# JuliaLinearAlgebra/AlgebraicMultigrid.jl

Hardware: AMD Instinct MI355X
Metric: V-cycle unknowns/sec + fine-level SpMV GB/s (% HBM peak), 3-D Poisson 256^3 (higher is better)
Workload: dtype f64

## Files before the change

### algebraicmultigrid.jl_amd/_libs.py

```python
import ctypes as C
import os

_HERE = os.path.dirname(os.path.abspath(__file__))
SETUP_SO = os.path.join(_HERE, "libamgsetup.so")
HIP_SO = os.path.join(_HERE, "libamghip.so")
HIP_F32_SO = os.path.join(_HERE, "libamghip_f32.so")

i32p = C.POINTER(C.c_int32)
f64p = C.POINTER(C.c_double)
i64 = C.c_int64
vp = C.c_void_p


class AMGError(RuntimeError):
    pass


class amgs_options(C.Structure):
    _fields_ = [("theta", C.c_double), ("max_levels", C.c_int32), ("max_coarse", C.c_int32),
                ("hermitian", C.c_int32), ("sa_omega", C.c_double), ("sa_improve_iters", C.c_int32),
                ("sa_B_is_vector", C.c_int32)]


class amgh_smoother_t(C.Structure):
# ... 141 lines not shown
    L.amgh_dev_upload.argtypes = [C.c_int, vp, vp, i64]
    L.amgh_dev_download.argtypes = [C.c_int, vp, vp, i64]
    L.amgh_dev_sync.argtypes = [C.c_int]
    L.amgh_stream.restype = vp
    L.amgh_stream.argtypes = [vp]
    L.amgh_timer_begin.argtypes = [vp]
    L.amgh_timer_end.argtypes = [vp, C.POINTER(C.c_double)]
    L.amgh_bench_op.argtypes = [vp, C.c_int, C.c_int, C.c_int, C.c_int, C.POINTER(C.c_double)]
    L.amgh_debug_chain_timing.argtypes = [C.c_int, vp]
    L.amgh_debug_merged_sweep_host.argtypes = [i64, i64, vp, vp, vp, C.c_int, C.c_int, C.c_double, vp, vp]
    L.amgh_debug_bw_poll_giveups.argtypes = [vp, C.c_int]
    L.amgh_debug_bw_mode.argtypes = [vp, C.c_int]
    L.amgh_debug_bw_dict.argtypes = [vp, C.c_int]
    L.amgh_debug_bw_late.argtypes = [vp, C.c_int]
    L.amgh_debug_coded_ops.argtypes = [vp, C.c_int]
    L.amgh_debug_set_sell_stream.argtypes = [C.c_int, i64, C.c_int]
    L.amgh_debug_sell_stream_launches.argtypes = [vp, C.c_int, C.c_int]
    L.amgh_debug_sell_stream_padded.argtypes = [vp, C.c_int, C.c_int]
    L.amgh_debug_sell_stream_padded.restype = i64
    L.amgh_debug_csr_sell.argtypes = [vp, C.c_int]
    L.amgh_debug_csr_sell.restype = i64
    L.amgh_debug_csr_sell_launches.argtypes = [vp]
    L.amgh_debug_csr_sell_apply.argtypes = [vp, C.c_int, vp, vp, vp]
    L.amgh_debug_bw_sweep_host.argtypes = [i64, vp, vp, vp, C.c_int, C.c_int, C.c_double, vp, vp, vp]
    L.amgh_debug_bw_dict_sweep_host.argtypes = [i64, vp, vp, vp, C.c_int, C.c_int, vp, vp, vp]
    L.amgh_debug_set_tunable.argtypes = [C.c_char_p, C.c_int]
    L.amgh_debug_get_tunable.argtypes = [C.c_char_p, C.POINTER(C.c_int)]
    L.amgh_profile_enable.argtypes = [vp, C.c_int]
    L.amgh_profile_read.argtypes = [vp, vp, C.c_int]
    L.amgh_set_use_graph.argtypes = [vp, C.c_int]


def _bind_dist(L):
    i64p = C.POINTER(i64)
    L.amgh_dist_rccl_available.argtypes = []
    L.amgh_dist_unique_id.argtypes = [vp]
    L.amgh_dist_create_rccl.argtypes = [C.POINTER(vp), C.c_int, C.c_int, C.c_int, vp]
    L.amgh_local_group_create.argtypes = [C.POINTER(vp), C.c_int]
    L.amgh_local_group_destroy.argtypes = [vp]
    L.amgh_local_group_destroy.restype = None
    L.amgh_local_group_abort.argtypes = [vp]
    L.amgh_local_group_abort.restype = None
    L.amgh_dist_create_local.argtypes = [C.POINTER(vp), C.c_int, C.c_int, vp]
    L.amgh_dist_create_ipc.argtypes = [C.POINTER(vp), C.c_int, C.c_int, C.c_int, C.c_char_p]
    L.amgh_dist_destroy.argtypes = [vp]
    L.amgh_dist_destroy.restype = None
# ... 93 lines not shown
```

### algebraicmultigrid.jl_amd/csrc/hip/amghip.hip

```cpp
#include "amghip_internal.hpp"
#include "gs_schedule.hpp"
#include "csr_ops.hpp"
#include "chebyshev.hpp"
#include "gmres_kernels.hpp"
#include "pcg_block_kernels.hpp"
#include "dist_pcg_kernels.hpp"

namespace {

constexpr int64_t kGraphAutoRows = 65536;

struct Level {
  int64_t n = 0, nc = 0;
  amgh_csr A, S, P, R;
  bool has_S = false;
  amgh_smoother_t pre{}, post{};
  real *res = nullptr, *cx = nullptr, *cb = nullptr, *tmp = nullptr;
  real* cheb_d = nullptr;
  ChebSide cheb[2];
  const ChebSide& cheb_of(const amgh_smoother_t& s) const { return &s == &post ? cheb[1] : cheb[0]; }
  real* il = nullptr;
  amgh_csr* smat() { return has_S ? &S : &A; }
  amgh_csr Pp, Rp;
  bool lo_ok = false;
// ... 1306 lines not shown
      if (!L->lo_ok || !L->Rp.rowptr || L->Rp.nrows < (1 << 18)) continue;
      if (hipMemsetAsync(L->res, 0, sizeof(real) * L->n, h->stream) != hipSuccess) return -1001;
      double ms[2] = {0, 0};
      int rc = AMGH_OK;
      for (int v = 0; v < 2 && rc == AMGH_OK; ++v) {
        L->Rp.xcd_map = v == 1;
        rc = csr_apply(&L->Rp, M_SPMV, L->res, nullptr, L->cb, h->stream, 1);
        if (rc == AMGH_OK && hipEventRecord(h->t0, h->stream) != hipSuccess) rc = -1001;
        for (int r = 0; r < 4 && rc == AMGH_OK; ++r) rc = csr_apply(&L->Rp, M_SPMV, L->res, nullptr, L->cb, h->stream, 1);
        float t = 0.f;
        if (rc == AMGH_OK && (hipEventRecord(h->t1, h->stream) != hipSuccess || hipEventSynchronize(h->t1) != hipSuccess ||
                              hipEventElapsedTime(&t, h->t0, h->t1) != hipSuccess)) rc = -1001;
        ms[v] = t;
      }
      L->Rp.xcd_map = false;
      RC_TRY(rc);
      L->Rp.xcd_map = ms[1] < 0.93 * ms[0];
      if (getenv("AMGH_VERBOSE")) fprintf(stderr, "[amghip] n=%lld restriction: %.3f ms, XCD-contiguous %.3f ms -> %s\n", (long long)L->n, ms[0] / 4, ms[1] / 4, L->Rp.xcd_map ? "XCD-contiguous" : "plain");
    }
  if (h->nrhs == 1)
    for (Level* L : h->levels) {
      GsSchedule* g = L->smat()->gs;
      const bool cd = g_stream_code != 0;
      if (!(L->lo_ok && g && g->nblk == 0)) {
        for (amgh_csr* M : {&L->A, &L->R, &L->P})
          if (M->rowptr) { RC_TRY(sell_build(M->rowptr, cd ? M->cc.ccol : nullptr, M->col, M->val, M->nrows, M->nnz, &M->sc, h->stream)); ws += M->sc.bytes; }
        continue;
      }
      if (!g->rowptr || g->compacted) continue;
      RC_TRY(sell_build(g->rowptr, cd ? L->lo_cc.ccol : nullptr, g->col, L->lo_val ? L->lo_val : g->val, L->n, g->nnz, &L->lo_sc, h->stream));
      RC_TRY(sell_build(L->Rp.rowptr, cd ? L->Rp.cc.ccol : nullptr, L->Rp.col, L->Rp.val, L->Rp.nrows, L->Rp.nnz, &L->Rp.sc, h->stream));
      RC_TRY(sell_build(L->Pp.rowptr, cd ? L->Pp.cc.ccol : nullptr, L->Pp.col, L->Pp.val, L->Pp.nrows, L->Pp.nnz, &L->Pp.sc, h->stream));
      if (L->n >= (1 << 18) && g_sell_min_rows >= ((int64_t)1 << 18)) {
        real* ty = nullptr;
        RC_TRY(dev_alloc(&ty, L->n));
        int rc = AMGH_OK;
        if (hipMemsetAsync(ty, 0, sizeof(real) * L->n, h->stream) != hipSuccess || hipMemsetAsync(L->res, 0, sizeof(real) * L->n, h->stream) != hipSuccess ||
            hipMemsetAsync(L->cx, 0, sizeof(real) * L->nc, h->stream) != hipSuccess) rc = -1001;
        const real* val = L->lo_val ? L->lo_val : g->val;
        auto run = [&](int which) -> int {
          if (which == AMGH_OP_A) return raw_apply(M_RESID, g->rowptr, g->col, val, L->n, L->res, L->n, L->res, L->n, ty, L->n, h->stream, 1, &L->lo_cc, &L->lo_sc);
          if (which == AMGH_OP_R) return csr_apply(&L->Rp, M_SPMV, L->res, nullptr, L->cb, h->stream, 1, true);
          return raw_apply(M_ADD, L->Pp.rowptr, L->Pp.col, L->Pp.val, L->n, L->cx, L->nc, nullptr, 0, ty, L->n, h->stream, 1, &L->Pp.cc, &L->Pp.sc);
        };
        const int keep = g_sell_stream;
        for (int which : {AMGH_OP_A, AMGH_OP_R, AMGH_OP_P}) {
          SellCols* sc = which == AMGH_OP_A ? &L->lo_sc : which == AMGH_OP_R ? &L->Rp.sc : &L->Pp.sc;
          if (!sc->w || (which == AMGH_OP_R ? L->Rp.nrows : L->n) < (1 << 18)) continue;
          double ms[2] = {0, 0};
          for (int v = 0; v < 2 && rc == AMGH_OK; ++v) {
            g_sell_stream = v;
            rc = run(which);
            if (rc == AMGH_OK && hipEventRecord(h->t0, h->stream) != hipSuccess) rc = -1001;
            for (int r = 0; r < 4 && rc == AMGH_OK; ++r) rc = run(which);
            float t = 0.f;
            if (rc == AMGH_OK && (hipEventRecord(h->t1, h->stream) != hipSuccess || hipEventSynchronize(h->t1) != hipSuccess ||
                                  hipEventElapsedTime(&t, h->t0, h->t1) != hipSuccess)) rc = -1001;
            ms[v] = t;
          }
          sc->launches = 0;
          if (rc != AMGH_OK) break;
          if (getenv("AMGH_VERBOSE")) fprintf(stderr, "[amghip] n=%lld operator %d: csr_stream_kernel %.3f ms, sliced-ELL %.3f ms\n", (long long)L->n, which, ms[0] / 4, ms[1] / 4);
          if (!(ms[1] < 0.97 * ms[0])) sc->free_dev();
        }
        g_sell_stream = keep;
        if (hipStreamSynchronize(h->stream) != hipSuccess && rc == AMGH_OK) rc = -1001;
        hipFree(ty);
        RC_TRY(rc);
      }
      ws += L->lo_sc.bytes + L->Rp.sc.bytes + L->Pp.sc.bytes;
      if (getenv("AMGH_VERBOSE"))
        fprintf(stderr, "[amghip] n=%lld sliced-ELL padded / entries: A %.3f  R %.3f  P %.3f (0: not taken)\n", (long long)L->n, (double)L->lo_sc.padded / std::max<int64_t>(1, g->nnz),
                (double)L->Rp.sc.padded / std::max<int64_t>(1, L->Rp.nnz), (double)L->Pp.sc.padded / std::max<int64_t>(1, L->Pp.nnz));
    }
  if (gs_trim() && g_stream_code && g_trim_coded) {
    HIP_TRY(hipStreamSynchronize(h->stream));
    for (Level* L : h->levels) {
      for (amgh_csr* M : {&L->Rp, &L->Pp})
        if (M->cc.ccol && M->col && M->val) {
          hipFree(M->col); hipFree(M->val); M->col = nullptr; M->val = nullptr;
          M->bytes -= M->nnz * kEntB;
        }
      amgh_csr* S = L->smat();
      GsSchedule* g = S->gs;
      if (L->lo_cc.ccol && g && g->bw.on && g->bw.flow.on && !g->bw.rec && g->segs.empty() && !g->mf && !g->mb && g->col && g->val) {
        hipFree(g->col); hipFree(g->val); g->col = nullptr; g->val = nullptr;
// ... 1059 lines not shown
  return sc ? (sc->w ? sc->padded : 0) : -1;
}

int64_t amgh_debug_csr_sell(amgh_csr_t* op, int coded) {
  if (!op) return AMGH_EINVAL;
  HIP_TRY(hipSetDevice(op->device));
  if (coded && !op->cc.ccol) {
    RC_TRY(code_values(op->col, op->val, op->nrows, op->ncols, op->nnz, &op->cc, nullptr, 1));
    op->bytes += op->cc.bytes;
  }
  RC_TRY(sell_build(op->rowptr, coded ? op->cc.ccol : nullptr, op->col, op->val, op->nrows, op->nnz, &op->sc, nullptr));
  op->bytes += op->sc.bytes;
  return op->sc.w ? op->sc.padded : 0;
}
int amgh_debug_csr_sell_apply(amgh_csr_t* op, int mode, const real* x_d, const real* b_d, real* y_d) {
  if (!op || !x_d || !y_d || mode < M_SPMV || mode > M_ADD || (mode == M_RESID && !b_d)) return AMGH_EINVAL;
  HIP_TRY(hipSetDevice(op->device));
  RC_TRY(csr_apply(op, mode, x_d, b_d, y_d, nullptr, 1, true));
  HIP_TRY(hipDeviceSynchronize());
  return AMGH_OK;
}
int amgh_debug_csr_sell_launches(const amgh_csr_t* op) { return op ? (int)(op->sc.launches & 0x7fffffffu) : -1; }

int amgh_debug_chain_timing(int enable, unsigned long long* out8) {
  if (enable && !g_chain_tim) {
    HIP_TRY(hipMalloc((void**)&g_chain_tim, 8 * sizeof(unsigned long long)));
    HIP_TRY(hipMemset(g_chain_tim, 0, 8 * sizeof(unsigned long long)));
  }
  if (out8 && g_chain_tim) {
    HIP_TRY(hipDeviceSynchronize());
    HIP_TRY(hipMemcpy(out8, g_chain_tim, 8 * sizeof(unsigned long long), hipMemcpyDeviceToHost));
    HIP_TRY(hipMemset(g_chain_tim, 0, 8 * sizeof(unsigned long long)));
  }
  if (!enable && g_chain_tim) { hipFree(g_chain_tim); g_chain_tim = nullptr; }
  return AMGH_OK;
}

int amgh_profile_enable(amgh_t* h, int on) {
  if (!h) return AMGH_EINVAL;
  h->profile = on != 0;
  return AMGH_OK;
}
int amgh_profile_read(amgh_t* h, double* out, int reset) {
  if (!h || !out) return AMGH_EINVAL;
  RC_TRY(prof_flush(h));
  const int L1 = (int)h->levels.size() + 1;
// ... 19 lines not shown
```

### algebraicmultigrid.jl_amd/csrc/hip/amghip_internal.hpp

```cpp
#pragma once
#include "amghip_kernels.hpp"
#include "gs_blocks.hpp"
#include "gs_flow.hpp"

#include <algorithm>
#include <chrono>
#include <cmath>
#include <cstdio>
#include <cstring>
#include <atomic>
#include <mutex>
#include <string>
#include <system_error>
#include <thread>
#include <utility>
#include <vector>

#include "../../../include/amghip.h"

using namespace amgh;

#define HIP_TRY(expr)                                   \
  do {                                                  \
    hipError_t e_ = (expr);                             \
// ... 280 lines not shown
    hipFree(bw.flow.fd); hipFree(bw.flow.srec); hipFree(bw.flow.aux); hipFree(bw.flow.fl_mb); hipFree(bw.flow.fl_slot); hipFree(bw.flow.mbox);
    hipFree(bw.flow.xaux); hipFree(bw.flow.xfl_mb); hipFree(bw.flow.xfl_slot); hipFree(bw.flow.xlist);
    hipFree(bw.flow.crec); hipFree(bw.flow.dict); hipFree(bw.flow.dict_ent);
    bw = Bw();
    hipFree(d_lvl_ptr); hipFree(rowptr); hipFree(col); hipFree(val);
    hipFree(perm); hipFree(dpos); if (!diag_shared) hipFree(diag);
    hipFree(rowmeta); hipFree(desc); hipFree(bp); hipFree(xp); hipFree(permx);
    d_lvl_ptr = rowptr = col = perm = dpos = nullptr; val = diag = bp = xp = nullptr; rowmeta = desc = nullptr; permx = nullptr;
  }
};

}

#include "dev_scan.hpp"

struct CodedCols {
  uint32_t* ccol = nullptr; real* vtab = nullptr; int n = 0;
  int64_t bytes = 0;
  void free_dev() { hipFree(ccol); hipFree(vtab); ccol = nullptr; vtab = nullptr; n = 0; bytes = 0; }
};

constexpr int kSellCapPct = 130, kSellCapPlainPct = 110;
constexpr int kSellLongSteps = 12;
struct SellCols {
  uint32_t* w = nullptr; real* v = nullptr; uint2* slice = nullptr; uint8_t* len8 = nullptr;
  int64_t nslices = 0, padded = 0, bytes = 0;
  unsigned launches = 0;
  void free_dev() { hipFree(w); hipFree(v); hipFree(slice); hipFree(len8); w = nullptr; v = nullptr; slice = nullptr; len8 = nullptr; nslices = padded = bytes = 0; }
};

struct amgh_csr {
  CodedCols cc;
  SellCols sc;
  bool cc_tried = false;
  bool xcd_map = false;
  int device = 0;
  int64_t nrows = 0, ncols = 0, nnz = 0;
  int32_t* rowptr = nullptr;
  int32_t* col = nullptr;
  real* val = nullptr;
  int32_t* dpos = nullptr;
  real* diag = nullptr;
  GsSchedule* gs = nullptr;
  int gs_nrhs_hint = 0;
  uint32_t pipe_epoch = 0; const void* pipe_rmbox = nullptr; int pipe_grid = 0;
  int64_t bytes = 0;
};

namespace {

int g_gs_block_pipe = 1;
// ... 2 lines not shown
int g_gs_bigslot = 1;
int g_gs_merge = 16;
int g_jacobi_zero = 1;
int g_rhs_il = 1;
int g_gs_tiny = 1;
int g_gs_wave_quad = 1;
int g_gs_bw = 1;
int g_gs_bw_rows = 512;
int g_gs_bw_flow = 1;
int g_gs_bw_spin = 0;
int g_gs_bw_skip_pub = -1;
int g_gs_bw_nc = -1;
int g_gs_bw_nrhs = 1;
int g_gs_bw_chain = 1;
int g_stream_code = 1;
int g_trim_coded = 1;
int g_gs_bw_inorder = 0;
int g_gs_bw_dict = 1;
int g_gs_bw_relay = 3;
int g_gs_flow_xzero = 1;
int g_gs_flow_perm_io = 1;
int g_sell_stream = 1;
int64_t g_sell_min_rows = (int64_t)1 << 18;
int g_sell_cap_pct = 0;
unsigned int g_perm_io_sweeps[2] = {0, 0};
int g_gs_bw_two_min_rows = 200000;
int g_gs_sell = 1;
int g_gs_lean = -1;
int g_gs_ept = 0;
int g_gs_lpr = 0;
int g_gs_il = 1;
int g_pcg_fused = 1;
int g_tail_dense_rows = 6144;
int g_tail_dense = 1;
int g_gs_dense_blk = 4096;
int g_gs_dense_tri = 1;
int g_gs_block_inverse = 1;

std::atomic<unsigned long long> g_sched_epoch{0};

unsigned long long* g_chain_tim = nullptr;

constexpr int kChainWidth = 1024;

__global__ void find_diag_kernel(const int32_t* rowptr, const int32_t* col, const real* val, int n,
                                 int32_t* dpos, real* diag) {
// ... 58 lines not shown
```

### algebraicmultigrid.jl_amd/csrc/hip/amghip_kernels.hpp

```cpp
#pragma once
#include <hip/hip_runtime.h>
#include <stdint.h>

#ifndef AMGH_REAL
#define AMGH_REAL double
#endif

namespace amgh {

using real = AMGH_REAL;

constexpr int kWave = 64;
constexpr int kThreads = 256;
constexpr int kNumXcd = 8;

enum StreamMode : int {
  M_SPMV = 0,
  M_RESID = 1,
  M_ADD = 2,
  M_JACOBI = 3,
  M_GS = 4,
  M_SOR = 5,
  M_CHEB1 = 6,
  M_CHEB = 7
// ... 251 lines not shown
          a.y[i] = (gb[q] - acc[q]) / d;
        } else {
          a.y[i] = (1.0 - a.omega) * a.y[i] + (a.omega / d) * (gb[q] - acc[q]);
        }
      }
    }
  }
}

using DefaultCfg = StreamCfg<1024, 1024, 8192, 4, false, false>;

struct SellStreamArgs {
  const uint32_t* w;
  const real* v;
  const uint2* slice;
  const uint8_t* len;
  const int32_t* rowptr;
  const real* vtab;
  int32_t vtab_n;
  int32_t nrows, nslices;
  const real* x;
  const real* b;
  real* y;
};
template <int MODE, bool CODED, int B>
__global__ __launch_bounds__(kThreads) void sell_stream_kernel(SellStreamArgs a) {
  static_assert(MODE == M_SPMV || MODE == M_RESID || MODE == M_ADD, "SpMV-type passes only");
  __shared__ real s_tab[CODED ? kCodeMax : 1];
  if (CODED) {
    if ((int)threadIdx.x < a.vtab_n) s_tab[threadIdx.x] = a.vtab[threadIdx.x];
    __syncthreads();
  }
  const int s = (int)blockIdx.x * (kThreads / kWave) + __builtin_amdgcn_readfirstlane((int)(threadIdx.x >> 6));
  if (s >= a.nslices) return;
  const int lane = threadIdx.x & (kWave - 1);
  const int r = s * kWave + lane;
  const bool live = r < a.nrows;
  int len = 0;
  if (live) len = a.len ? (int)a.len[r] : a.rowptr[r + 1] - a.rowptr[r];
  const uint2 sd = a.slice[s];
  const int nit = (int)sd.y;
  const int64_t base = (int64_t)sd.x * kWave + lane;
  uint32_t w[B];
  real v[B];
#pragma unroll
  for (int e = 0; e < B; ++e) {
    w[e] = 0; v[e] = 0.0;
    if (e < nit) { w[e] = a.w[base + (int64_t)e * kWave]; if (!CODED) v[e] = a.v[base + (int64_t)e * kWave]; }
  }
  real acc = 0.0;
  for (int t = 0; t < nit; t += B) {
    uint32_t wn[B];
    real vn[B];
#pragma unroll
    for (int e = 0; e < B; ++e) {
      wn[e] = 0; vn[e] = 0.0;
      if (t + B + e < nit) { wn[e] = a.w[base + (int64_t)(t + B + e) * kWave]; if (!CODED) vn[e] = a.v[base + (int64_t)(t + B + e) * kWave]; }
    }
    real xv[B];
#pragma unroll
    for (int e = 0; e < B; ++e) {
      const uint32_t c = CODED ? (w[e] & ((1u << kCodeBits) - 1)) : w[e];
      xv[e] = t + e < len ? a.x[c] : (real)0.0;
      if (CODED) v[e] = s_tab[w[e] >> kCodeBits];
    }
#pragma unroll
    for (int e = 0; e < B; ++e)
      if (t + e < len) acc = acc + v[e] * xv[e];
#pragma unroll
    for (int e = 0; e < B; ++e) { w[e] = wn[e]; v[e] = vn[e]; }
  }
  if (!live) return;
  if (MODE == M_SPMV) a.y[r] = acc;
  else if (MODE == M_RESID) a.y[r] = a.b[r] - acc;
  else a.y[r] = a.y[r] + acc;
}
__global__ void sell_steps_kernel(const int32_t* rowptr, int nrows, int nslices, int32_t* steps) {
  const int s = blockIdx.x * blockDim.x + threadIdx.x;
  if (s >= nslices) return;
  const int r1 = min(s * kWave + kWave, nrows);
  int m = 0;
  for (int r = s * kWave; r < r1; ++r) m = max(m, rowptr[r + 1] - rowptr[r]);
  steps[s] = m;
}
__global__ void sell_stream_fill_kernel(const int32_t* rowptr, const uint32_t* w_in, const real* v_in, const uint2* slice, int nrows,
                                        int nslices, uint32_t* w, real* v, uint8_t* len8) {
  const int64_t gid = (int64_t)blockIdx.x * blockDim.x + threadIdx.x;
  const int s = (int)(gid >> 6), lane = (int)(gid & 63);
  if (s >= nslices) return;
  const uint2 sd = slice[s];
  const int r = s * kWave + lane;
  int32_t a0 = 0, len = 0;
  if (r < nrows) { a0 = rowptr[r]; len = rowptr[r + 1] - a0; if (len8) len8[r] = (uint8_t)len; }
  const int64_t base = (int64_t)sd.x * kWave + lane;
  for (int t = 0; t < (int)sd.y; ++t) {
    w[base + (int64_t)t * kWave] = t < len ? w_in[a0 + t] : 0u;
    if (v) v[base + (int64_t)t * kWave] = t < len ? v_in[a0 + t] : (real)0.0;
  }
}

__device__ __forceinline__ real seq_sum_range(const real* s, int lo, int hi, real acc) {
  int j = lo;
  if (hi - j >= 8) {
    real p[8], q[8];
#pragma unroll
    for (int e = 0; e < 8; ++e) p[e] = s[j + e];
    j += 8;
    while (hi - j >= 16) {
#pragma unroll
      for (int e = 0; e < 8; ++e) q[e] = s[j + e];
#pragma unroll
      for (int e = 0; e < 8; ++e) acc += p[e];
#pragma unroll
      for (int e = 0; e < 8; ++e) p[e] = s[j + 8 + e];
#pragma unroll
      for (int e = 0; e < 8; ++e) acc += q[e];
// ... 1656 lines not shown
```

### algebraicmultigrid.jl_amd/csrc/hip/csr_ops.hpp

```cpp
#pragma once
#include <atomic>

namespace {


template <int MODE, class CFG = DefaultCfg, bool CODED = false>
int launch_stream(const StreamArgs& a0, hipStream_t st, int ncolv = 1) {
  const int nrows = a0.row_end - a0.row_begin;
  if (nrows <= 0) return AMGH_OK;
  StreamArgs a = a0;
  a.ncolv = ncolv;
  const int nb = (nrows + CFG::ROWS - 1) / CFG::ROWS;
  const int64_t grid = (CFG::XCD || ncolv > 1) ? (int64_t)((nb + kNumXcd - 1) / kNumXcd) * kNumXcd * ncolv : nb;
  hipLaunchKernelGGL((csr_stream_kernel<MODE, CFG, CODED>), dim3((unsigned)grid), dim3(CFG::THREADS), 0, st, a);
  HIP_TRY(hipGetLastError());
  return AMGH_OK;
}

constexpr int kGsBlockTarget = 256;
constexpr int kGsMinRows = 4;
constexpr int kGsNnzPerWg = 256;
template <int MODE>
int launch_gs_level(const StreamArgs& a, int rows, hipStream_t st, int ncolv = 1) {
  const int width = a.row_end - a.row_begin;
// ... 88 lines not shown
    tab.erase(std::unique(tab.begin(), tab.end()), tab.end());
    if ((int)tab.size() > kCodeMax) ok = false;
    if (pass == 7) ok = false;
  }
  if (rc == AMGH_OK && ok && !tab.empty()) {
    std::vector<real> tv(tab.size());
    for (size_t i = 0; i < tab.size(); ++i) std::memcpy(&tv[i], &tab[i], sizeof(real));
    rc = dev_alloc(&out->ccol, nnz + 4);
    if (rc == AMGH_OK) rc = dev_alloc(&out->vtab, kCodeMax);
    if (rc == AMGH_OK && hipMemcpyAsync(d_tab, tv.data(), sizeof(real) * tv.size(), hipMemcpyHostToDevice, st) != hipSuccess) rc = -1001;
    if (rc == AMGH_OK && hipMemcpyAsync(out->vtab, tv.data(), sizeof(real) * tv.size(), hipMemcpyHostToDevice, st) != hipSuccess) rc = -1001;
    if (rc == AMGH_OK) {
      hipLaunchKernelGGL(code_encode_kernel, dim3((unsigned)std::min<int64_t>((nnz + 255) / 256, 8192)), dim3(256), 0, st, col, val, nnz, (const real*)d_tab, (int)tab.size(), out->ccol);
      if (hipGetLastError() != hipSuccess || hipStreamSynchronize(st) != hipSuccess) rc = -1001;
    }
    if (rc == AMGH_OK) { out->n = (int)tab.size(); out->bytes = nnz * 4 + kCodeMax * kRealB; }
    else out->free_dev();
  }
  hipFree(d_cnt); hipFree(d_miss); hipFree(d_tab);
  if (rc == AMGH_ENOMEM) { (void)hipGetLastError(); out->free_dev(); return AMGH_OK; }
  return rc;
}

int sell_build(const int32_t* rowptr, const uint32_t* ccol, const int32_t* col, const real* val, int64_t nrows, int64_t nnz,
               SellCols* out, hipStream_t st) {
  if (out->w || nrows < g_sell_min_rows || nrows <= 0 || nnz <= 0 || !rowptr || (!ccol && !(col && val))) return AMGH_OK;
  const int64_t ns = (nrows + kWave - 1) / kWave;
  int32_t* d_steps = nullptr;
  RC_TRY(dev_alloc(&d_steps, ns));
  hipLaunchKernelGGL(sell_steps_kernel, dim3((unsigned)((ns + 255) / 256)), dim3(256), 0, st, rowptr, (int)nrows, (int)ns, d_steps);
  std::vector<int32_t> steps((size_t)ns);
  if (hipMemcpyAsync(steps.data(), d_steps, sizeof(int32_t) * ns, hipMemcpyDeviceToHost, st) != hipSuccess || hipStreamSynchronize(st) != hipSuccess) { hipFree(d_steps); return -1001; }
  hipFree(d_steps);
  std::vector<uint2> sd((size_t)ns);
  int64_t off = 0;
  int longest = 0;
  for (int64_t s = 0; s < ns; ++s) { sd[(size_t)s] = make_uint2((unsigned)off, (unsigned)steps[(size_t)s]); off += steps[(size_t)s]; longest = std::max(longest, steps[(size_t)s]); }
  const int64_t padded = off * kWave;
  const bool coded = ccol != nullptr;
  if (off >= ((int64_t)1 << 32) || padded * 100 > nnz * (int64_t)(g_sell_cap_pct > 0 ? g_sell_cap_pct : coded ? kSellCapPct : kSellCapPlainPct)) return AMGH_OK;
  int rc = dev_alloc(&out->w, padded);
  if (rc == AMGH_OK && !coded) rc = dev_alloc(&out->v, padded);
  if (rc == AMGH_OK) rc = dev_alloc(&out->slice, ns);
  if (rc == AMGH_OK && longest <= 255) rc = dev_alloc(&out->len8, nrows);
  if (rc == AMGH_OK && hipMemcpyAsync(out->slice, sd.data(), sizeof(uint2) * ns, hipMemcpyHostToDevice, st) != hipSuccess) rc = -1001;
  if (rc == AMGH_OK) {
    hipLaunchKernelGGL(sell_stream_fill_kernel, dim3((unsigned)((ns * kWave + 255) / 256)), dim3(256), 0, st, rowptr,
                       coded ? ccol : (const uint32_t*)col, coded ? (const real*)nullptr : val, (const uint2*)out->slice, (int)nrows, (int)ns,
                       out->w, out->v, out->len8);
    if (hipGetLastError() != hipSuccess || hipStreamSynchronize(st) != hipSuccess) rc = -1001;
  }
  if (rc != AMGH_OK) { out->free_dev(); if (rc == AMGH_ENOMEM) { (void)hipGetLastError(); return AMGH_OK; } return rc; }
  out->nslices = ns; out->padded = padded;
  out->bytes = padded * (coded ? 4 : kEntB) + ns * 8 + (out->len8 ? nrows : 0);
  return AMGH_OK;
}
bool sell_apply(int mode, const StreamArgs& a, const SellCols* sc, hipStream_t st, int ncolv, int* rc) {
  if (!sc || !sc->w || !g_sell_stream || ncolv != 1 || (!sc->v && !a.vtab)) return false;
  SellStreamArgs s{};
  s.w = sc->w; s.v = sc->v; s.slice = sc->slice; s.len = sc->len8; s.rowptr = a.rowptr; s.vtab = a.vtab; s.vtab_n = a.vtab_n;
  s.nrows = a.row_end; s.nslices = (int32_t)sc->nslices; s.x = a.x; s.b = a.b; s.y = a.y;
  const dim3 grid((unsigned)((sc->nslices + kThreads / kWave - 1) / (kThreads / kWave))), block(kThreads);
  const bool coded = sc->v == nullptr;
  const bool b8 = coded && sc->padded >= (int64_t)kSellLongSteps * kWave * sc->nslices;
#define AMGH_SELL_LAUNCH(M) \
  do { \
    if (b8) hipLaunchKernelGGL((sell_stream_kernel<M, true, 8>), grid, block, 0, st, s); \
    else if (coded) hipLaunchKernelGGL((sell_stream_kernel<M, true, 4>), grid, block, 0, st, s); \
    else hipLaunchKernelGGL((sell_stream_kernel<M, false, 4>), grid, block, 0, st, s); \
  } while (0)
  switch (mode) {
    case M_SPMV: AMGH_SELL_LAUNCH(M_SPMV); break;
    case M_RESID: AMGH_SELL_LAUNCH(M_RESID); break;
    case M_ADD: AMGH_SELL_LAUNCH(M_ADD); break;
    default: return false;
  }
#undef AMGH_SELL_LAUNCH
  ++const_cast<SellCols*>(sc)->launches;
  *rc = hipGetLastError() == hipSuccess ? AMGH_OK : -1001;
  return true;
}

int csr_apply(const amgh_csr* op, int mode, const real* x, const real* b, real* y, hipStream_t st,
              int ncolv = 1, bool sell = false) {
  StreamArgs a{};
  a.rowptr = op->rowptr; a.col = op->col; a.val = op->val;
  a.ccol = op->cc.ccol; a.vtab = op->cc.vtab; a.vtab_n = op->cc.n;
  a.x = x; a.y = y; a.b = b;
  a.row_begin = 0; a.row_end = (int32_t)op->nrows;
  a.ldx = op->ncols; a.ldy = op->nrows; a.ldb = op->nrows;
  int rc = AMGH_OK;
  if (sell && sell_apply(mode, a, &op->sc, st, ncolv, &rc)) return rc;
  switch (mode) {
    case M_SPMV: return launch_stream_sized<M_SPMV>(a, st, ncolv, op->xcd_map);
    case M_RESID: return launch_stream_sized<M_RESID>(a, st, ncolv);
    case M_ADD: return launch_stream_sized<M_ADD>(a, st, ncolv);
  }
  return AMGH_EINVAL;
}
// ... 719 lines not shown
```

### include/amghip.h

```cpp
#ifndef AMGHIP_H
#define AMGHIP_H

#include <stdint.h>

#ifdef __cplusplus
extern "C" {
#endif

#ifndef AMGH_REAL
#define AMGH_REAL double
#endif
typedef AMGH_REAL amgh_real;

typedef struct amgh_handle amgh_t;
typedef struct amgh_csr amgh_csr_t;

#define AMGH_OK 0
#define AMGH_EINVAL (-2)
#define AMGH_ESTATE (-3)
#define AMGH_ENOMEM (-4)
#define AMGH_EUNSUPPORTED (-5)

enum { AMGH_SMOOTH_NONE = 0, AMGH_SMOOTH_GS = 1, AMGH_SMOOTH_JACOBI = 2, AMGH_SMOOTH_SOR = 3, AMGH_SMOOTH_CHEBYSHEV = 4 };
enum { AMGH_SWEEP_FORWARD = 0, AMGH_SWEEP_BACKWARD = 1, AMGH_SWEEP_SYMMETRIC = 2 };
// ... 218 lines not shown

int amgh_debug_bw_dict_sweep_host(int64_t nrows, const int32_t* rowptr, const int32_t* col, const amgh_real* val, int target_rows,
                                  int backward, amgh_real* x, const amgh_real* b, int64_t* stats5);

int amgh_debug_bw_poll_giveups(const amgh_t* h, int l);

int amgh_debug_bw_mode(const amgh_t* h, int l);
int amgh_debug_bw_dict(const amgh_t* h, int l);
int amgh_debug_bw_late(const amgh_t* h, int l);
int amgh_debug_coded_ops(const amgh_t* h, int l);

int amgh_debug_set_tunable(const char* name, int value);
int amgh_debug_get_tunable(const char* name, int* value);
int amgh_debug_set_perm_io(int on);
int amgh_debug_get_perm_io(void);
int amgh_debug_perm_io_sweeps(int which);
int amgh_debug_set_sell_stream(int on, int64_t min_rows, int cap_pct);
int amgh_debug_get_sell_stream(void);
int amgh_debug_sell_stream_launches(const amgh_t* h, int level, int which);
int64_t amgh_debug_sell_stream_padded(const amgh_t* h, int level, int which);
int64_t amgh_debug_csr_sell(amgh_csr_t* op, int coded);
int amgh_debug_csr_sell_apply(amgh_csr_t* op, int mode, const amgh_real* x_d, const amgh_real* b_d, amgh_real* y_d);
int amgh_debug_csr_sell_launches(const amgh_csr_t* op);

int amgh_set_use_graph(amgh_t* h, int on);

#ifdef __cplusplus
}
#endif
#endif
```

Measured before the change: 1.227 billion.

## Add row-reordered sliced-ELL variants chosen by setup-time timing

Adds sorted row orderings for the sliced-ELL SpMV format: sorting rows by length within windows (to cut padding) and sorting restriction rows by minimum column (for x locality). The kernel reads a per-slot row id map. During setup the sorted copy is timed against the natural copy and the CSR kernel, and the fastest is kept. This adds build cost, map reads in the kernel and scattered output writes in exchange for less padding or better gather locality.

```diff
diff --git a/algebraicmultigrid.jl_amd/_libs.py b/algebraicmultigrid.jl_amd/_libs.py
--- a/algebraicmultigrid.jl_amd/_libs.py
+++ b/algebraicmultigrid.jl_amd/_libs.py
@@ -187,6 +187,10 @@
     L.amgh_debug_csr_sell.restype = i64
     L.amgh_debug_csr_sell_launches.argtypes = [vp]
     L.amgh_debug_csr_sell_apply.argtypes = [vp, C.c_int, vp, vp, vp]
+    L.amgh_debug_set_sell_order.argtypes = [C.c_int, i64]
+    L.amgh_debug_sell_order.argtypes = [vp, C.c_int, C.c_int]
+    L.amgh_debug_csr_sell_ordered.argtypes = [vp, C.c_int, C.c_int, C.c_int]
+    L.amgh_debug_csr_sell_ordered.restype = i64
     L.amgh_debug_bw_sweep_host.argtypes = [i64, vp, vp, vp, C.c_int, C.c_int, C.c_double, vp, vp, vp]
     L.amgh_debug_bw_dict_sweep_host.argtypes = [i64, vp, vp, vp, C.c_int, C.c_int, vp, vp, vp]
     L.amgh_debug_set_tunable.argtypes = [C.c_char_p, C.c_int]
diff --git a/algebraicmultigrid.jl_amd/csrc/hip/amghip.hip b/algebraicmultigrid.jl_amd/csrc/hip/amghip.hip
--- a/algebraicmultigrid.jl_amd/csrc/hip/amghip.hip
+++ b/algebraicmultigrid.jl_amd/csrc/hip/amghip.hip
@@ -1352,46 +1352,84 @@
     for (Level* L : h->levels) {
       GsSchedule* g = L->smat()->gs;
       const bool cd = g_stream_code != 0;
+      auto build_op = [&](const int32_t* rowptr, const uint32_t* ccol, const int32_t* col, const real* val, int64_t nrows, int64_t nnz, SellCols* sc, int which) -> int {
+        const bool forced = g_sell_order == 1 && nrows >= g_sell_order_min_rows;
+        if (forced && which == AMGH_OP_R) RC_TRY(sell_build(rowptr, ccol, col, val, nrows, nnz, sc, h->stream, g_sell_order_min_rows, kSellMapCol));
+        RC_TRY(sell_build(rowptr, ccol, col, val, nrows, nnz, sc, h->stream));
+        if (forced && which != AMGH_OP_R) RC_TRY(sell_build(rowptr, ccol, col, val, nrows, nnz, sc, h->stream, g_sell_order_min_rows, kSellMapLen));
+        return AMGH_OK;
+      };
       if (!(L->lo_ok && g && g->nblk == 0)) {
         for (amgh_csr* M : {&L->A, &L->R, &L->P})
-          if (M->rowptr) { RC_TRY(sell_build(M->rowptr, cd ? M->cc.ccol : nullptr, M->col, M->val, M->nrows, M->nnz, &M->sc, h->stream)); ws += M->sc.bytes; }
+          if (M->rowptr) {
+            RC_TRY(build_op(M->rowptr, cd ? M->cc.ccol : nullptr, M->col, M->val, M->nrows, M->nnz, &M->sc, M == &L->A ? AMGH_OP_A : M == &L->R ? AMGH_OP_R : AMGH_OP_P));
+            ws += M->sc.bytes;
+          }
         continue;
       }
       if (!g->rowptr || g->compacted) continue;
-      RC_TRY(sell_build(g->rowptr, cd ? L->lo_cc.ccol : nullptr, g->col, L->lo_val ? L->lo_val : g->val, L->n, g->nnz, &L->lo_sc, h->stream));
-      RC_TRY(sell_build(L->Rp.rowptr, cd ? L->Rp.cc.ccol : nullptr, L->Rp.col, L->Rp.val, L->Rp.nrows, L->Rp.nnz, &L->Rp.sc, h->stream));
-      RC_TRY(sell_build(L->Pp.rowptr, cd ? L->Pp.cc.ccol : nullptr, L->Pp.col, L->Pp.val, L->Pp.nrows, L->Pp.nnz, &L->Pp.sc, h->stream));
-      if (L->n >= (1 << 18) && g_sell_min_rows >= ((int64_t)1 << 18)) {
+      const bool timed = L->n >= (1 << 18) && g_sell_min_rows >= ((int64_t)1 << 18);
+      const real* val = L->lo_val ? L->lo_val : g->val;
+      struct Cand { const int32_t* rowptr; const uint32_t* ccol; const int32_t* col; const real* val; int64_t nrows, nnz; SellCols* sc; };
+      const Cand cand[3] = {{g->rowptr, cd ? L->lo_cc.ccol : nullptr, g->col, val, L->n, g->nnz, &L->lo_sc},
+                            {L->Pp.rowptr, cd ? L->Pp.cc.ccol : nullptr, L->Pp.col, L->Pp.val, L->Pp.nrows, L->Pp.nnz, &L->Pp.sc},
+                            {L->Rp.rowptr, cd ? L->Rp.cc.ccol : nullptr, L->Rp.col, L->Rp.val, L->Rp.nrows, L->Rp.nnz, &L->Rp.sc}};
+      for (int which : {AMGH_OP_A, AMGH_OP_R, AMGH_OP_P}) {
+        const Cand& c = cand[which];
+        if (timed) RC_TRY(sell_build(c.rowptr, c.ccol, c.col, c.val, c.nrows, c.nnz, c.sc, h->stream, which == AMGH_OP_R ? 1 : -1));
+        else RC_TRY(build_op(c.rowptr, c.ccol, c.col, c.val, c.nrows, c.nnz, c.sc, which));
+      }
+      if (timed) {
         real* ty = nullptr;
         RC_TRY(dev_alloc(&ty, L->n));
         int rc = AMGH_OK;
         if (hipMemsetAsync(ty, 0, sizeof(real) * L->n, h->stream) != hipSuccess || hipMemsetAsync(L->res, 0, sizeof(real) * L->n, h->stream) != hipSuccess ||
             hipMemsetAsync(L->cx, 0, sizeof(real) * L->nc, h->stream) != hipSuccess) rc = -1001;
-        const real* val = L->lo_val ? L->lo_val : g->val;
         auto run = [&](int which) -> int {
           if (which == AMGH_OP_A) return raw_apply(M_RESID, g->rowptr, g->col, val, L->n, L->res, L->n, L->res, L->n, ty, L->n, h->stream, 1, &L->lo_cc, &L->lo_sc);
           if (which == AMGH_OP_R) return csr_apply(&L->Rp, M_SPMV, L->res, nullptr, L->cb, h->stream, 1, true);
           return raw_apply(M_ADD, L->Pp.rowptr, L->Pp.col, L->Pp.val, L->n, L->cx, L->nc, nullptr, 0, ty, L->n, h->stream, 1, &L->Pp.cc, &L->Pp.sc);
         };
+        auto time4 = [&](int which, double* ms) -> int {
+          int r = run(which);
+          if (r == AMGH_OK && hipEventRecord(h->t0, h->stream) != hipSuccess) r = -1001;
+          for (int k = 0; k < 4 && r == AMGH_OK; ++k) r = run(which);
+          float t = 0.f;
+          if (r == AMGH_OK && (hipEventRecord(h->t1, h->stream) != hipSuccess || hipEventSynchronize(h->t1) != hipSuccess ||
+                               hipEventElapsedTime(&t, h->t0, h->t1) != hipSuccess)) r = -1001;
+          *ms = t;
+          return r;
+        };
         const int keep = g_sell_stream;
         for (int which : {AMGH_OP_A, AMGH_OP_R, AMGH_OP_P}) {
-          SellCols* sc = which == AMGH_OP_A ? &L->lo_sc : which == AMGH_OP_R ? &L->Rp.sc : &L->Pp.sc;
-          if (!sc->w || (which == AMGH_OP_R ? L->Rp.nrows : L->n) < (1 << 18)) continue;
-          double ms[2] = {0, 0};
-          for (int v = 0; v < 2 && rc == AMGH_OK; ++v) {
-            g_sell_stream = v;
-            rc = run(which);
-            if (rc == AMGH_OK && hipEventRecord(h->t0, h->stream) != hipSuccess) rc = -1001;
-            for (int r = 0; r < 4 && rc == AMGH_OK; ++r) rc = run(which);
-            float t = 0.f;
-            if (rc == AMGH_OK && (hipEventRecord(h->t1, h->stream) != hipSuccess || hipEventSynchronize(h->t1) != hipSuccess ||
-                                  hipEventElapsedTime(&t, h->t0, h->t1) != hipSuccess)) rc = -1001;
-            ms[v] = t;
+          const Cand& c = cand[which];
+          SellCols* sc = c.sc;
+          SellCols so;
+          if (g_sell_order == -1 && rc == AMGH_OK) {
+            if (which == AMGH_OP_R) rc = sell_build(c.rowptr, c.ccol, c.col, c.val, c.nrows, c.nnz, &so, h->stream, 1, kSellMapCol);
+            else if (!sc->w) rc = sell_build(c.rowptr, c.ccol, c.col, c.val, c.nrows, c.nnz, &so, h->stream, -1, kSellMapLen);
           }
+          if (rc != AMGH_OK) break;
+          if (!sc->w && !so.w) continue;
+          double ms[3] = {0, 0, 0};
+          g_sell_stream = 0;
+          rc = time4(which, &ms[0]);
+          g_sell_stream = 1;
+          if (rc == AMGH_OK && sc->w) rc = time4(which, &ms[1]);
+          if (rc == AMGH_OK && so.w) { std::swap(*sc, so); rc = time4(which, &ms[2]); std::swap(*sc, so); }
+          if (rc != AMGH_OK) { so.free_dev(); break; }
+          const bool nat = sc->w != nullptr, srt = so.w != nullptr;
+          const bool take_srt = srt && ms[2] < 0.97 * ms[0] && (!nat || ms[2] < 0.97 * ms[1]);
+          const bool take_nat = !take_srt && nat && ms[1] < 0.97 * ms[0];
+          if (getenv("AMGH_VERBOSE")) {
+            fprintf(stderr, "[amghip] n=%lld operator %d: csr_stream_kernel %.3f ms, sliced-ELL %.3f ms", (long long)L->n, which, ms[0] / 4, ms[1] / 4);
+            if (srt) fprintf(stderr, ", %s order (padded / entries %.3f) %.3f ms", so.order == kSellMapCol ? "column" : "length", (double)so.padded / std::max<int64_t>(1, c.nnz), ms[2] / 4);
+            fprintf(stderr, " (0: no such copy) -> %s\n", take_srt ? "sorted copy" : take_nat ? "natural copy" : "csr_stream_kernel");
+          }
+          if (take_srt) std::swap(*sc, so);
+          else if (!take_nat) sc->free_dev();
+          so.free_dev();
           sc->launches = 0;
-          if (rc != AMGH_OK) break;
-          if (getenv("AMGH_VERBOSE")) fprintf(stderr, "[amghip] n=%lld operator %d: csr_stream_kernel %.3f ms, sliced-ELL %.3f ms\n", (long long)L->n, which, ms[0] / 4, ms[1] / 4);
-          if (!(ms[1] < 0.97 * ms[0])) sc->free_dev();
         }
         g_sell_stream = keep;
         if (hipStreamSynchronize(h->stream) != hipSuccess && rc == AMGH_OK) rc = -1001;
@@ -2497,6 +2535,32 @@
 }
 int amgh_debug_csr_sell_launches(const amgh_csr_t* op) { return op ? (int)(op->sc.launches & 0x7fffffffu) : -1; }
 
+int amgh_debug_set_sell_order(int mode, int64_t min_rows) {
+  if (mode < -1 || mode > 1) return AMGH_EINVAL;
+  g_sell_order = mode;
+  g_sell_order_min_rows = min_rows > 0 ? min_rows : (int64_t)1 << 18;
+  return AMGH_OK;
+}
+int amgh_debug_get_sell_order(void) { return g_sell_order; }
+int amgh_debug_sell_order(const amgh_t* h, int level, int which) {
+  const SellCols* sc = sell_of(h, level, which);
+  return sc ? (sc->w ? sc->order : 0) : -1;
+}
+int64_t amgh_debug_csr_sell_ordered(amgh_csr_t* op, int coded, int order, int window) {
+  if (!op) return AMGH_EINVAL;
+  HIP_TRY(hipSetDevice(op->device));
+  if (coded && !op->cc.ccol) {
+    RC_TRY(code_values(op->col, op->val, op->nrows, op->ncols, op->nnz, &op->cc, nullptr, 1));
+    op->bytes += op->cc.bytes;
+  }
+  HIP_TRY(hipDeviceSynchronize());
+  op->bytes -= op->sc.bytes;
+  op->sc.free_dev();
+  RC_TRY(sell_build(op->rowptr, coded ? op->cc.ccol : nullptr, op->col, op->val, op->nrows, op->nnz, &op->sc, nullptr, -1, order, window, true));
+  op->bytes += op->sc.bytes;
+  return op->sc.w ? op->sc.padded : 0;
+}
+
 int amgh_debug_chain_timing(int enable, unsigned long long* out8) {
   if (enable && !g_chain_tim) {
     HIP_TRY(hipMalloc((void**)&g_chain_tim, 8 * sizeof(unsigned long long)));
diff --git a/algebraicmultigrid.jl_amd/csrc/hip/amghip_internal.hpp b/algebraicmultigrid.jl_amd/csrc/hip/amghip_internal.hpp
--- a/algebraicmultigrid.jl_amd/csrc/hip/amghip_internal.hpp
+++ b/algebraicmultigrid.jl_amd/csrc/hip/amghip_internal.hpp
@@ -326,11 +326,17 @@
 
 constexpr int kSellCapPct = 130, kSellCapPlainPct = 110;
 constexpr int kSellLongSteps = 12;
+constexpr int kSellWindow = 256;
 struct SellCols {
   uint32_t* w = nullptr; real* v = nullptr; uint2* slice = nullptr; uint8_t* len8 = nullptr;
+  void* rowid = nullptr;
+  int order = 0, window = 0;
   int64_t nslices = 0, padded = 0, bytes = 0;
   unsigned launches = 0;
-  void free_dev() { hipFree(w); hipFree(v); hipFree(slice); hipFree(len8); w = nullptr; v = nullptr; slice = nullptr; len8 = nullptr; nslices = padded = bytes = 0; }
+  void free_dev() {
+    hipFree(w); hipFree(v); hipFree(slice); hipFree(len8); hipFree(rowid);
+    w = nullptr; v = nullptr; slice = nullptr; len8 = nullptr; rowid = nullptr; order = window = 0; nslices = padded = bytes = 0;
+  }
 };
 
 struct amgh_csr {
@@ -379,6 +385,8 @@
 int g_gs_flow_perm_io = 1;
 int g_sell_stream = 1;
 int64_t g_sell_min_rows = (int64_t)1 << 18;
+int g_sell_order = -1;
+int64_t g_sell_order_min_rows = (int64_t)1 << 18;
 int g_sell_cap_pct = 0;
 unsigned int g_perm_io_sweeps[2] = {0, 0};
 int g_gs_bw_two_min_rows = 200000;
diff --git a/algebraicmultigrid.jl_amd/csrc/hip/amghip_kernels.hpp b/algebraicmultigrid.jl_amd/csrc/hip/amghip_kernels.hpp
--- a/algebraicmultigrid.jl_amd/csrc/hip/amghip_kernels.hpp
+++ b/algebraicmultigrid.jl_amd/csrc/hip/amghip_kernels.hpp
@@ -297,8 +297,25 @@
   const real* x;
   const real* b;
   real* y;
+  const void* rowid;
+  int32_t window;
 };
-template <int MODE, bool CODED, int B>
+constexpr int kSellMapNone = 0, kSellMapLen = 1, kSellMapCol = 2;
+constexpr unsigned kSellDead16 = 0xFFFFu;
+template <int MAP>
+__device__ __forceinline__ int sell_slot_row(const void* rowid, int window, int slot, int nrows) {
+  if (MAP == kSellMapNone) return slot < nrows ? slot : -1;
+  if (MAP == kSellMapLen) {
+    const unsigned q = ((const uint16_t*)rowid)[slot];
+    return q == kSellDead16 ? -1 : (slot & ~(window - 1)) + (int)q;
+  }
+  return ((const int32_t*)rowid)[slot];
+}
+__device__ __forceinline__ int sell_slot_row(int map, const void* rowid, int window, int slot, int nrows) {
+  return map == kSellMapLen ? sell_slot_row<kSellMapLen>(rowid, window, slot, nrows)
+         : map == kSellMapCol ? sell_slot_row<kSellMapCol>(rowid, window, slot, nrows) : sell_slot_row<kSellMapNone>(rowid, window, slot, nrows);
+}
+template <int MODE, bool CODED, int B, int MAP = kSellMapNone>
 __global__ __launch_bounds__(kThreads) void sell_stream_kernel(SellStreamArgs a) {
   static_assert(MODE == M_SPMV || MODE == M_RESID || MODE == M_ADD, "SpMV-type passes only");
   __shared__ real s_tab[CODED ? kCodeMax : 1];
@@ -309,10 +326,11 @@
   const int s = (int)blockIdx.x * (kThreads / kWave) + __builtin_amdgcn_readfirstlane((int)(threadIdx.x >> 6));
   if (s >= a.nslices) return;
   const int lane = threadIdx.x & (kWave - 1);
-  const int r = s * kWave + lane;
-  const bool live = r < a.nrows;
+  const int slot = s * kWave + lane;
+  const int r = sell_slot_row<MAP>(a.rowid, a.window, slot, a.nrows);
+  const bool live = r >= 0;
   int len = 0;
-  if (live) len = a.len ? (int)a.len[r] : a.rowptr[r + 1] - a.rowptr[r];
+  if (live) len = a.len ? (int)a.len[MAP == kSellMapNone ? r : slot] : a.rowptr[r + 1] - a.rowptr[r];
   const uint2 sd = a.slice[s];
   const int nit = (int)sd.y;
   const int64_t base = (int64_t)sd.x * kWave + lane;
@@ -350,23 +368,56 @@
   else if (MODE == M_RESID) a.y[r] = a.b[r] - acc;
   else a.y[r] = a.y[r] + acc;
 }
-__global__ void sell_steps_kernel(const int32_t* rowptr, int nrows, int nslices, int32_t* steps) {
+constexpr int kSellWindowMax = 4096;
+__global__ __launch_bounds__(kThreads) void sell_len_order_kernel(const int32_t* rowptr, int nrows, int window, uint16_t* rowid) {
+  __shared__ int32_t s_len[kSellWindowMax];
+  const int r0 = (int)blockIdx.x * window;
+  const int m = min(window, nrows - r0);
+  for (int i = threadIdx.x; i < m; i += kThreads) s_len[i] = rowptr[r0 + i + 1] - rowptr[r0 + i];
+  __syncthreads();
+  const int mslots = (m + kWave - 1) & ~(kWave - 1);
+  for (int i = m + (int)threadIdx.x; i < mslots; i += kThreads) rowid[r0 + i] = (uint16_t)kSellDead16;
+  for (int i = threadIdx.x; i < m; i += kThreads) {
+    const int li = s_len[i];
+    int before = 0;
+    for (int j = 0; j < m; ++j) {
+      const int lj = s_len[j];
+      before += (lj > li || (lj == li && j < i)) ? 1 : 0;
+    }
+    rowid[r0 + before] = (uint16_t)i;
+  }
+}
+__global__ void sell_min_col_kernel(const int32_t* rowptr, const uint32_t* w_in, uint32_t mask, int nrows, uint32_t* key, int32_t* row) {
+  const int r = blockIdx.x * blockDim.x + threadIdx.x;
+  if (r >= nrows) return;
+  uint32_t m = 0xFFFFFFFFu;
+  for (int k = rowptr[r]; k < rowptr[r + 1]; ++k) m = min(m, w_in[k] & mask);
+  key[r] = m;
+  row[r] = r;
+}
+__global__ void sell_steps_kernel(const int32_t* rowptr, int nrows, int nslices, int32_t* steps, int map = kSellMapNone,
+                                  const void* rowid = nullptr, int window = 0) {
   const int s = blockIdx.x * blockDim.x + threadIdx.x;
   if (s >= nslices) return;
-  const int r1 = min(s * kWave + kWave, nrows);
   int m = 0;
-  for (int r = s * kWave; r < r1; ++r) m = max(m, rowptr[r + 1] - rowptr[r]);
+  for (int slot = s * kWave; slot < s * kWave + kWave; ++slot) {
+    const int r = sell_slot_row(map, rowid, window, slot, nrows);
+    if (r >= 0) m = max(m, rowptr[r + 1] - rowptr[r]);
+  }
   steps[s] = m;
 }
 __global__ void sell_stream_fill_kernel(const int32_t* rowptr, const uint32_t* w_in, const real* v_in, const uint2* slice, int nrows,
-                                        int nslices, uint32_t* w, real* v, uint8_t* len8) {
+                                        int nslices, uint32_t* w, real* v, uint8_t* len8, int map = kSellMapNone,
+                                        const void* rowid = nullptr, int window = 0) {
   const int64_t gid = (int64_t)blockIdx.x * blockDim.x + threadIdx.x;
   const int s = (int)(gid >> 6), lane = (int)(gid & 63);
   if (s >= nslices) return;
   const uint2 sd = slice[s];
-  const int r = s * kWave + lane;
+  const int slot = s * kWave + lane;
+  const int r = sell_slot_row(map, rowid, window, slot, nrows);
   int32_t a0 = 0, len = 0;
-  if (r < nrows) { a0 = rowptr[r]; len = rowptr[r + 1] - a0; if (len8) len8[r] = (uint8_t)len; }
+  if (r >= 0) { a0 = rowptr[r]; len = rowptr[r + 1] - a0; }
+  if (len8 && (map != kSellMapNone || r >= 0)) len8[map == kSellMapNone ? r : slot] = (uint8_t)len;
   const int64_t base = (int64_t)sd.x * kWave + lane;
   for (int t = 0; t < (int)sd.y; ++t) {
     w[base + (int64_t)t * kWave] = t < len ? w_in[a0 + t] : 0u;
diff --git a/algebraicmultigrid.jl_amd/csrc/hip/csr_ops.hpp b/algebraicmultigrid.jl_amd/csrc/hip/csr_ops.hpp
--- a/algebraicmultigrid.jl_amd/csrc/hip/csr_ops.hpp
+++ b/algebraicmultigrid.jl_amd/csrc/hip/csr_ops.hpp
@@ -1,5 +1,6 @@
 #pragma once
 #include <atomic>
+#include <rocprim/rocprim.hpp>
 
 namespace {
 
@@ -134,37 +135,84 @@
   return rc;
 }
 
+int sell_col_order(const int32_t* rowptr, const uint32_t* w_in, bool coded, int64_t nrows, int64_t nslots, int32_t* map, hipStream_t st) {
+  uint32_t *key = nullptr, *key_out = nullptr;
+  int32_t* row = nullptr;
+  void* tmp = nullptr;
+  size_t tmp_bytes = 0;
+  int rc = dev_alloc(&key, nrows);
+  if (rc == AMGH_OK) rc = dev_alloc(&key_out, nrows);
+  if (rc == AMGH_OK) rc = dev_alloc(&row, nrows);
+  if (rc == AMGH_OK) {
+    hipLaunchKernelGGL(sell_min_col_kernel, dim3((unsigned)((nrows + 255) / 256)), dim3(256), 0, st, rowptr, w_in,
+                       coded ? (1u << kCodeBits) - 1 : 0xFFFFFFFFu, (int)nrows, key, row);
+    if (hipGetLastError() != hipSuccess) rc = -1001;
+  }
+  if (rc == AMGH_OK && rocprim::radix_sort_pairs(nullptr, tmp_bytes, key, key_out, row, map, (size_t)nrows, 0u, 32u, st) != hipSuccess) rc = -1001;
+  if (rc == AMGH_OK && hipMalloc(&tmp, std::max<size_t>(tmp_bytes, 16)) != hipSuccess) rc = AMGH_ENOMEM;
+  if (rc == AMGH_OK && rocprim::radix_sort_pairs(tmp, tmp_bytes, key, key_out, row, map, (size_t)nrows, 0u, 32u, st) != hipSuccess) rc = -1001;
+  if (rc == AMGH_OK && nslots > nrows && hipMemsetAsync(map + nrows, 0xFF, sizeof(int32_t) * (nslots - nrows), st) != hipSuccess) rc = -1001;
+  if (hipStreamSynchronize(st) != hipSuccess && rc == AMGH_OK) rc = -1001;
+  hipFree(tmp); hipFree(key); hipFree(key_out); hipFree(row);
+  return rc;
+}
 int sell_build(const int32_t* rowptr, const uint32_t* ccol, const int32_t* col, const real* val, int64_t nrows, int64_t nnz,
-               SellCols* out, hipStream_t st) {
-  if (out->w || nrows < g_sell_min_rows || nrows <= 0 || nnz <= 0 || !rowptr || (!ccol && !(col && val))) return AMGH_OK;
+               SellCols* out, hipStream_t st, int64_t min_rows = -1, int order = kSellMapNone, int window = 0, bool force = false) {
+  if (min_rows < 0) min_rows = g_sell_min_rows;
+  if (out->w || (!force && nrows < min_rows) || nrows <= 0 || nnz <= 0 || !rowptr || (!ccol && !(col && val))) return AMGH_OK;
+  if (order == kSellMapLen && window <= 0) {
+    const char* e = getenv("AMGH_SELL_WINDOW");
+    window = e ? atoi(e) : kSellWindow;
+  }
+  if (order < kSellMapNone || order > kSellMapCol ||
+      (order == kSellMapLen && (window < kWave || window > kSellWindowMax || (window & (window - 1))))) return AMGH_EINVAL;
   const int64_t ns = (nrows + kWave - 1) / kWave;
+  const bool coded = ccol != nullptr;
+  const uint32_t* w_in = coded ? ccol : (const uint32_t*)col;
+  void* d_map = nullptr;
+  int rc = AMGH_OK;
+  if (order == kSellMapLen) {
+    uint16_t* m16 = nullptr;
+    rc = dev_alloc(&m16, ns * kWave);
+    d_map = m16;
+    if (rc == AMGH_OK) hipLaunchKernelGGL(sell_len_order_kernel, dim3((unsigned)((nrows + window - 1) / window)), dim3(kThreads), 0, st, rowptr, (int)nrows, window, m16);
+  } else if (order == kSellMapCol) {
+    int32_t* m32 = nullptr;
+    rc = dev_alloc(&m32, ns * kWave);
+    d_map = m32;
+    if (rc == AMGH_OK) rc = sell_col_order(rowptr, w_in, coded, nrows, ns * kWave, m32, st);
+  }
   int32_t* d_steps = nullptr;
-  RC_TRY(dev_alloc(&d_steps, ns));
-  hipLaunchKernelGGL(sell_steps_kernel, dim3((unsigned)((ns + 255) / 256)), dim3(256), 0, st, rowptr, (int)nrows, (int)ns, d_steps);
+  if (rc == AMGH_OK) rc = dev_alloc(&d_steps, ns);
   std::vector<int32_t> steps((size_t)ns);
-  if (hipMemcpyAsync(steps.data(), d_steps, sizeof(int32_t) * ns, hipMemcpyDeviceToHost, st) != hipSuccess || hipStreamSynchronize(st) != hipSuccess) { hipFree(d_steps); return -1001; }
+  if (rc == AMGH_OK) {
+    hipLaunchKernelGGL(sell_steps_kernel, dim3((unsigned)((ns + 255) / 256)), dim3(256), 0, st, rowptr, (int)nrows, (int)ns, d_steps, order, (const void*)d_map, window);
+    if (hipMemcpyAsync(steps.data(), d_steps, sizeof(int32_t) * ns, hipMemcpyDeviceToHost, st) != hipSuccess || hipStreamSynchronize(st) != hipSuccess) rc = -1001;
+  }
   hipFree(d_steps);
+  if (rc != AMGH_OK) { hipFree(d_map); if (rc == AMGH_ENOMEM) { (void)hipGetLastError(); return AMGH_OK; } return rc; }
   std::vector<uint2> sd((size_t)ns);
   int64_t off = 0;
   int longest = 0;
   for (int64_t s = 0; s < ns; ++s) { sd[(size_t)s] = make_uint2((unsigned)off, (unsigned)steps[(size_t)s]); off += steps[(size_t)s]; longest = std::max(longest, steps[(size_t)s]); }
   const int64_t padded = off * kWave;
-  const bool coded = ccol != nullptr;
-  if (off >= ((int64_t)1 << 32) || padded * 100 > nnz * (int64_t)(g_sell_cap_pct > 0 ? g_sell_cap_pct : coded ? kSellCapPct : kSellCapPlainPct)) return AMGH_OK;
-  int rc = dev_alloc(&out->w, padded);
+  if (off >= ((int64_t)1 << 32) || (!force && padded * 100 > nnz * (int64_t)(g_sell_cap_pct > 0 ? g_sell_cap_pct : coded ? kSellCapPct : kSellCapPlainPct))) { hipFree(d_map); return AMGH_OK; }
+  const int64_t nlen = order == kSellMapNone ? nrows : ns * kWave;
+  rc = dev_alloc(&out->w, padded);
   if (rc == AMGH_OK && !coded) rc = dev_alloc(&out->v, padded);
   if (rc == AMGH_OK) rc = dev_alloc(&out->slice, ns);
-  if (rc == AMGH_OK && longest <= 255) rc = dev_alloc(&out->len8, nrows);
+  if (rc == AMGH_OK && longest <= 255) rc = dev_alloc(&out->len8, nlen);
   if (rc == AMGH_OK && hipMemcpyAsync(out->slice, sd.data(), sizeof(uint2) * ns, hipMemcpyHostToDevice, st) != hipSuccess) rc = -1001;
   if (rc == AMGH_OK) {
     hipLaunchKernelGGL(sell_stream_fill_kernel, dim3((unsigned)((ns * kWave + 255) / 256)), dim3(256), 0, st, rowptr,
-                       coded ? ccol : (const uint32_t*)col, coded ? (const real*)nullptr : val, (const uint2*)out->slice, (int)nrows, (int)ns,
-                       out->w, out->v, out->len8);
+                       w_in, coded ? (const real*)nullptr : val, (const uint2*)out->slice, (int)nrows, (int)ns,
+                       out->w, out->v, out->len8, order, (const void*)d_map, window);
     if (hipGetLastError() != hipSuccess || hipStreamSynchronize(st) != hipSuccess) rc = -1001;
   }
-  if (rc != AMGH_OK) { out->free_dev(); if (rc == AMGH_ENOMEM) { (void)hipGetLastError(); return AMGH_OK; } return rc; }
+  if (rc != AMGH_OK) { out->free_dev(); hipFree(d_map); if (rc == AMGH_ENOMEM) { (void)hipGetLastError(); return AMGH_OK; } return rc; }
   out->nslices = ns; out->padded = padded;
-  out->bytes = padded * (coded ? 4 : kEntB) + ns * 8 + (out->len8 ? nrows : 0);
+  out->rowid = d_map; out->order = order; out->window = order == kSellMapLen ? window : 0;
+  out->bytes = padded * (coded ? 4 : kEntB) + ns * 8 + (out->len8 ? nlen : 0) + (order == kSellMapLen ? 2 : order == kSellMapCol ? 4 : 0) * ns * kWave;
   return AMGH_OK;
 }
 bool sell_apply(int mode, const StreamArgs& a, const SellCols* sc, hipStream_t st, int ncolv, int* rc) {
@@ -172,14 +220,21 @@
   SellStreamArgs s{};
   s.w = sc->w; s.v = sc->v; s.slice = sc->slice; s.len = sc->len8; s.rowptr = a.rowptr; s.vtab = a.vtab; s.vtab_n = a.vtab_n;
   s.nrows = a.row_end; s.nslices = (int32_t)sc->nslices; s.x = a.x; s.b = a.b; s.y = a.y;
+  s.rowid = sc->rowid; s.window = sc->window;
   const dim3 grid((unsigned)((sc->nslices + kThreads / kWave - 1) / (kThreads / kWave))), block(kThreads);
   const bool coded = sc->v == nullptr;
   const bool b8 = coded && sc->padded >= (int64_t)kSellLongSteps * kWave * sc->nslices;
+#define AMGH_SELL_LAUNCH_MAP(M, MAP) \
+  do { \
+    if (b8) hipLaunchKernelGGL((sell_stream_kernel<M, true, 8, MAP>), grid, block, 0, st, s); \
+    else if (coded) hipLaunchKernelGGL((sell_stream_kernel<M, true, 4, MAP>), grid, block, 0, st, s); \
+    else hipLaunchKernelGGL((sell_stream_kernel<M, false, 4, MAP>), grid, block, 0, st, s); \
+  } while (0)
 #define AMGH_SELL_LAUNCH(M) \
   do { \
-    if (b8) hipLaunchKernelGGL((sell_stream_kernel<M, true, 8>), grid, block, 0, st, s); \
-    else if (coded) hipLaunchKernelGGL((sell_stream_kernel<M, true, 4>), grid, block, 0, st, s); \
-    else hipLaunchKernelGGL((sell_stream_kernel<M, false, 4>), grid, block, 0, st, s); \
+    if (sc->order == kSellMapLen) AMGH_SELL_LAUNCH_MAP(M, kSellMapLen); \
+    else if (sc->order == kSellMapCol) AMGH_SELL_LAUNCH_MAP(M, kSellMapCol); \
+    else AMGH_SELL_LAUNCH_MAP(M, kSellMapNone); \
   } while (0)
   switch (mode) {
     case M_SPMV: AMGH_SELL_LAUNCH(M_SPMV); break;
@@ -187,6 +242,7 @@
     case M_ADD: AMGH_SELL_LAUNCH(M_ADD); break;
     default: return false;
   }
+#undef AMGH_SELL_LAUNCH_MAP
 #undef AMGH_SELL_LAUNCH
   ++const_cast<SellCols*>(sc)->launches;
   *rc = hipGetLastError() == hipSuccess ? AMGH_OK : -1001;
diff --git a/include/amghip.h b/include/amghip.h
--- a/include/amghip.h
+++ b/include/amghip.h
@@ -264,6 +264,10 @@
 int64_t amgh_debug_csr_sell(amgh_csr_t* op, int coded);
 int amgh_debug_csr_sell_apply(amgh_csr_t* op, int mode, const amgh_real* x_d, const amgh_real* b_d, amgh_real* y_d);
 int amgh_debug_csr_sell_launches(const amgh_csr_t* op);
+int amgh_debug_set_sell_order(int mode, int64_t min_rows);
+int amgh_debug_get_sell_order(void);
+int amgh_debug_sell_order(const amgh_t* h, int level, int which);
+int64_t amgh_debug_csr_sell_ordered(amgh_csr_t* op, int coded, int order, int window);
 
 int amgh_set_use_graph(amgh_t* h, int on);
 
```

After: 1.233 billion, median of 6. About the same (+0.4%).
